# lambdaclass/lambdaworks_kzg

Measured on AMD Instinct MI355X. Metric: blob_to_kzg_commitment ops/sec (4096-elem blobs), higher is better.
Workload: dtype u32

## Files before the change

### lambdaworks_kzg_amd/csrc/direct.hip

```cpp
#include <stdlib.h>
#include <chrono>
#include "kernels.h"
#include "knobs.h"

namespace lwk {

template <int C>
struct DirectPlan {
    static constexpr int NW = (255 + C - 1) / C;
    static constexpr int H = 1 << (C - 1);
    static constexpr int WTOP = 255 - C * (NW - 1);
    static constexpr int HTOP = 1 << WTOP;
    static constexpr size_t TOP_BASE = (size_t)(NW - 1) * kBlobElems * H;
    static constexpr size_t ENTRIES = TOP_BASE + (size_t)kBlobElems * HTOP;
};

struct DirectPlanRt {
    int c, nw, wtop;
    uint32_t h, htop;
    size_t top_base, entries;
};

static DirectPlanRt make_plan(int bits) {
    DirectPlanRt p{};
// ... 382 lines not shown
    asm volatile(
#include "direct_fold_asm.inc"
        :
        : "s"(src), "s"(out), "s"(flag), "s"(per), "v"(lane), "s"(levels)
        :
#include "direct_fold_asm_clobbers.inc"
    );
#endif
}

__global__ __launch_bounds__(64) void k_direct_fold_lanes_asm_alone(const uint32_t *__restrict__ lane_out, G1Xyzz29 *__restrict__ partials,
                                                                    uint32_t *__restrict__ redo, int lanes_per_block, int blocks_per_blob) {
#if defined(__HIP_DEVICE_COMPILE__)
    const uint32_t unit = blockIdx.x;
    uint32_t *flag = redo + unit / blocks_per_blob;
    if (*flag) return;
    const uint32_t *src = lane_out + (size_t)unit * lanes_per_block * kLaneWords;
    G1Xyzz29 *out = partials + unit;
    const uint32_t per = lanes_per_block / 64, lane = threadIdx.x, levels = 6;
    asm volatile(
#include "direct_fold_asm.inc"
        :
        : "s"(src), "s"(out), "s"(flag), "s"(per), "v"(lane), "s"(levels)
        :
#include "direct_fold_asm_clobbers_pad.inc"
    );
#endif
}

template <bool ALONE>
__global__ __launch_bounds__(64) void k_commit_tail(const uint32_t *__restrict__ lane_out, G1Xyzz29 *__restrict__ sums,
                                                    uint32_t *__restrict__ redo, uint8_t *__restrict__ out48, int lanes_per_block) {
#if defined(__HIP_DEVICE_COMPILE__)
    const uint32_t blob = blockIdx.x;
    uint32_t *flag = redo + blob;
    G1Xyzz29 *out = sums + blob;
    const uint32_t lane = threadIdx.x;
    __builtin_amdgcn_s_setprio(2);
    if (!*flag) {
        const uint32_t *src = lane_out + (size_t)blob * lanes_per_block * kLaneWords;
        const uint32_t per = lanes_per_block / 64, levels = 6;
        if (ALONE) {
            asm volatile(
#include "direct_fold_asm.inc"
                :
                : "s"(src), "s"(out), "s"(flag), "s"(per), "v"(lane), "s"(levels)
                :
#include "direct_fold_asm_clobbers_pad.inc"
            );
        } else {
            asm volatile(
#include "direct_fold_asm.inc"
                :
                : "s"(src), "s"(out), "s"(flag), "s"(per), "v"(lane), "s"(levels)
                :
#include "direct_fold_asm_clobbers.inc"
            );
        }
        if (__hip_atomic_load(flag, __ATOMIC_RELAXED, __HIP_MEMORY_SCOPE_AGENT)) {
            const FoldPoint acc = fold_lane_sums(src + (size_t)lane * kLaneWords, (int)lane, (int)per);
            if (lane == 0) *out = *(const G1Xyzz29 *)&acc;
            __builtin_amdgcn_fence(__ATOMIC_RELEASE, "agent");
        }
    }
    uint32_t w[12];
    g1_compress_words(w, *out);
    if (lane != 0) return;
    uint32_t *o = (uint32_t *)(out48 + 48 * (size_t)blob);
#pragma unroll
    for (int k = 0; k < 12; k++) o[k] = w[k];
#endif
}

__global__ __launch_bounds__(64) void k_direct_fold(const G1Xyzz29 *__restrict__ partials, G1Xyzz29 *__restrict__ sums,
                                                    int per_blob) {
    const size_t b = blockIdx.x;
    const int lane = threadIdx.x;
    __builtin_amdgcn_s_setprio(2);
    G1Xyzz29 s = lane < per_blob ? partials[b * per_blob + lane] : G1Xyzz29::infinity();
    s = wave_fold(s, lane);
    if (lane == 0) sums[b] = s;
}

struct CoopParams {
    uint32_t k[8];
    uint32_t pack;
    uint32_t wtop, row_bytes, n0;
    uint32_t part_words, ctr_words;
};

constexpr uint32_t kCoopUnitWords = 56;

static void coop_geometry(const DirectPlanRt &P, int rpq, uint32_t &n0, uint32_t &units, uint32_t &counters) {
    const uint32_t groups = (uint32_t)((P.nw + rpq - 1) / rpq);
    n0 = kBlobElems * groups / 16;
    units = 0;
    counters = 0;
    for (uint32_t n = n0; n > 1; n = (n + 15) / 16) {
        units += n;
        counters += (n + 15) / 16;
    }
}

__global__ __launch_bounds__(256) void k_coop_msm_asm(const uint64_t *__restrict__ win_dev, const uint4 *__restrict__ scalars,
                                                     uint32_t *__restrict__ partials, uint32_t *__restrict__ counters,
                                                     G1Xyzz29 *__restrict__ sums, uint32_t *__restrict__ redo, CoopParams prm) {
#if defined(__HIP_DEVICE_COMPILE__)
    const uint32_t blob = blockIdx.y, lane = threadIdx.x & 63;
    const uint32_t unit = blockIdx.x * 4 + __builtin_amdgcn_readfirstlane(threadIdx.x >> 6);
    const uint4 *sc = scalars + (size_t)blob * kBlobElems * 2;
    uint32_t *part = partials + (size_t)blob * prm.part_words;
    uint32_t *ctr = counters + (size_t)blob * prm.ctr_words;
    G1Xyzz29 *out = sums + blob;
    uint32_t *flag = redo + blob;
    asm volatile(
#include "coop_asm.inc"
        :
        : "s"(win_dev), "s"(sc), "s"(part), "s"(ctr), "s"(out), "s"(flag), "s"(prm.k[0]), "s"(prm.k[1]), "s"(prm.k[2]), "s"(prm.k[3]),
          "s"(prm.k[4]), "s"(prm.k[5]), "s"(prm.k[6]), "s"(prm.k[7]), "s"(prm.pack), "s"(prm.wtop), "s"(prm.row_bytes), "s"(prm.n0), "s"(unit),
          "v"(lane)
        :
#include "coop_asm_clobbers.inc"
    );
#endif
}

static int coop_max_blobs() { return knobs().coop == 0 ? 0 : knobs().coop_max; }
static int coop_rows_per_quad(int nw, size_t n_blobs) {
    const int env = knobs().coop_rpq < 0 ? 0 : knobs().coop_rpq > 32 ? 32 : knobs().coop_rpq;
    if (env) return env;
    const int groups = n_blobs >= 4 ? 1 : (int)(4 / n_blobs);
    return (nw + groups - 1) / groups;
}

constexpr int kRedoRows = 256;
static bool direct_asm_enabled() { return knobs().direct_asm; }

template <int CT>
static bool launch_direct_t(const DirectPlanRt &plan, const uint64_t *table, size_t row_bytes, const uint32_t *scalars_raw,
                            G1Xyzz29 *lane_scratch, G1Xyzz29 *partials, uint32_t *redo, G1Xyzz29 *sums, size_t n_blobs, hipStream_t st,
                            int fill, uint32_t *redo_flag_out, uint8_t *out48 = nullptr, bool redo_cleared = false) {
    const int kFillEnv = knobs().direct_fill;
    const int kFill = kFillEnv ? kFillEnv : fill ? fill : 512;
    CoopParams prm{};
    const int rpq = coop_rows_per_quad(plan.nw, n_blobs ? n_blobs : 1);
    uint32_t units = 0, counters = 0;
    coop_geometry(plan, rpq, prm.n0, units, counters);
    const bool coop_fits = units <= (uint32_t)kBlobElems && 1 + counters <= (uint32_t)kNumBuckets + 1;
    if ((int)n_blobs <= coop_max_blobs() && !fill && coop_fits) {
        for (int j = 0; j + 1 < plan.nw; j++) {
            const int bit = plan.c * j;
            const uint64_t v = (uint64_t)(plan.h - 1) << (bit & 31);
            uint64_t carry = v;
            for (int w = bit >> 5; w < 8 && carry; w++) {
                carry += prm.k[w];
                prm.k[w] = (uint32_t)carry;
                carry >>= 32;
            }
        }
        prm.pack = (uint32_t)plan.c | ((uint32_t)plan.nw << 8) | ((uint32_t)rpq << 16) | (12u << 24);
        prm.wtop = (uint32_t)plan.wtop;
        prm.row_bytes = (uint32_t)row_bytes;
        prm.part_words = units * kCoopUnitWords;
        prm.ctr_words = counters;
        uint32_t *ctr = redo + n_blobs;
        if (redo_flag_out) {
            ProfScope p("k_coop_msm_asm", st);
            hipLaunchKernelGGL(k_coop_msm_asm, dim3(prm.n0 / 4, (unsigned)n_blobs), dim3(256), 0, st, table, (const uint4 *)scalars_raw,
                               (uint32_t *)lane_scratch, ctr, sums, redo_flag_out, prm);
            return false;
        }
        hipMemsetAsync(redo, 0, n_blobs * (1 + (size_t)counters) * sizeof(uint32_t), st);
        {
            ProfScope p("k_coop_msm_asm", st);
            hipLaunchKernelGGL(k_coop_msm_asm, dim3(prm.n0 / 4, (unsigned)n_blobs), dim3(256), 0, st, table, (const uint4 *)scalars_raw,
                               (uint32_t *)lane_scratch, ctr, sums, redo, prm);
        }
        {
            ProfScope p("k_direct_redo", st);
            hipLaunchKernelGGL(k_direct_accumulate<CT>, dim3(1, (unsigned)n_blobs, 1), dim3(kDirThreads), 0, st, table,
                               (const uint4 *)scalars_raw, sums, kBlobElems / kDirThreads, plan, (uint32_t)row_bytes, (const uint32_t *)redo);
        }
        return false;
    }
    int blocks_per_blob = 1, wsplit = 1;
    while (blocks_per_blob < 16 && n_blobs * blocks_per_blob < (size_t)kFill) blocks_per_blob <<= 1;
    while (wsplit < 4 && n_blobs * blocks_per_blob * wsplit * 8 <= (size_t)kFill) wsplit <<= 1;
    const int scalars_per_lane = kBlobElems / (kDirThreads * blocks_per_blob);
    const int parts = blocks_per_blob * wsplit;
    G1Xyzz29 *dest = parts == 1 ? sums : partials;
    if (out48 && direct_asm_enabled() && wsplit == 1 && blocks_per_blob == 1 && knobs().fold_asm && knobs().commit_tail) {
        if (!redo_cleared) hipMemsetAsync(redo, 0, n_blobs * sizeof(uint32_t), st);
        {
            ProfScope p("k_direct_accumulate_asm", st);
            hipLaunchKernelGGL(k_direct_accumulate_asm, dim3(1, (unsigned)n_blobs), dim3(kDirThreads), 0, st, table, (const uint4 *)scalars_raw,
                               (uint32_t *)lane_scratch, redo, kBlobElems / kDirThreads, plan, (uint32_t)row_bytes);
        }
        {
            ProfScope p("k_direct_redo", st);
            const unsigned rows = n_blobs < (size_t)kRedoRows ? (unsigned)n_blobs : (unsigned)kRedoRows;
            hipLaunchKernelGGL(k_direct_second_pass<CT>, dim3(1, rows, 1), dim3(kDirThreads), 0, st, table, (const uint4 *)scalars_raw, sums,
                               plan, (uint32_t)row_bytes, (const uint32_t *)redo, (uint32_t)n_blobs);
        }
        {
            ProfScope p("k_commit_tail", st);
            if (n_blobs >= 1024 && !fill)
                hipLaunchKernelGGL(k_commit_tail<true>, dim3((unsigned)n_blobs), dim3(64), 0, st, (const uint32_t *)lane_scratch, sums, redo, out48,
                                   kDirThreads);
            else
                hipLaunchKernelGGL(k_commit_tail<false>, dim3((unsigned)n_blobs), dim3(64), 0, st, (const uint32_t *)lane_scratch, sums, redo, out48,
                                   kDirThreads);
        }
        return true;
    }
    if (direct_asm_enabled() && wsplit == 1) {
        const int threads = kDirThreads;
        hipMemsetAsync(redo, 0, n_blobs * sizeof(uint32_t), st);
        {
            ProfScope p("k_direct_accumulate_asm", st);
            hipLaunchKernelGGL(k_direct_accumulate_asm, dim3(blocks_per_blob, (unsigned)n_blobs), dim3(threads), 0, st, table,
                               (const uint4 *)scalars_raw, (uint32_t *)lane_scratch, redo, kBlobElems / (threads * blocks_per_blob), plan,
                               (uint32_t)row_bytes);
        }
        {
            ProfScope p("k_direct_fold_lanes", st);
            const int n_units = (int)n_blobs * blocks_per_blob;
            const bool fold_asm = knobs().fold_asm;
            if (fold_asm) {
                if (n_units >= 1024 && !fill)
                    hipLaunchKernelGGL(k_direct_fold_lanes_asm_alone, dim3((unsigned)n_units), dim3(64), 0, st, (const uint32_t *)lane_scratch,
                                       dest, redo, threads, blocks_per_blob);
                else
                    hipLaunchKernelGGL(k_direct_fold_lanes_asm, dim3((unsigned)n_units), dim3(64), 0, st, (const uint32_t *)lane_scratch, dest,
                                       redo, threads, blocks_per_blob);
            } else {
                hipLaunchKernelGGL(k_direct_fold_lanes, dim3((unsigned)n_units), dim3(64), 0, st, (const uint32_t *)lane_scratch, dest,
                                   (const uint32_t *)redo, threads, blocks_per_blob);
            }
        }
        {
            ProfScope p("k_direct_redo", st);
            hipLaunchKernelGGL(k_direct_accumulate<CT>, dim3(blocks_per_blob, (unsigned)n_blobs, 1), dim3(kDirThreads), 0, st, table,
                               (const uint4 *)scalars_raw, dest, scalars_per_lane, plan, (uint32_t)row_bytes, (const uint32_t *)redo);
        }
    } else {
        ProfScope p("k_direct_accumulate", st);
        hipLaunchKernelGGL(k_direct_accumulate<CT>, dim3(blocks_per_blob, (unsigned)n_blobs, wsplit), dim3(kDirThreads), 0, st,
                           table, (const uint4 *)scalars_raw, dest, scalars_per_lane, plan, (uint32_t)row_bytes, (const uint32_t *)nullptr);
    }
    if (parts > 1) {
        ProfScope p("k_direct_fold", st);
        hipLaunchKernelGGL(k_direct_fold, dim3((unsigned)n_blobs), dim3(64), 0, st, partials, sums, parts);
    }
    return false;
}


static bool launch_direct_any(int bits, const uint64_t *table, size_t row_bytes, const uint32_t *scalars_raw, G1Xyzz29 *lane_scratch,
                              G1Xyzz29 *partials, uint32_t *redo, G1Xyzz29 *sums, size_t n_blobs, hipStream_t st, int fill, uint32_t *redo_flag_out,
                              uint8_t *out48, bool redo_cleared) {
    const DirectPlanRt plan = make_plan(bits);
    if (!plan.entries) return false;
    switch (bits) {
        case 14: return launch_direct_t<14>(plan, table, row_bytes, scalars_raw, lane_scratch, partials, redo, sums, n_blobs, st, fill, redo_flag_out, out48, redo_cleared);
        case 15: return launch_direct_t<15>(plan, table, row_bytes, scalars_raw, lane_scratch, partials, redo, sums, n_blobs, st, fill, redo_flag_out, out48, redo_cleared);
        case 16: return launch_direct_t<16>(plan, table, row_bytes, scalars_raw, lane_scratch, partials, redo, sums, n_blobs, st, fill, redo_flag_out, out48, redo_cleared);
        default: return launch_direct_t<0>(plan, table, row_bytes, scalars_raw, lane_scratch, partials, redo, sums, n_blobs, st, fill, redo_flag_out, out48, redo_cleared);
    }
}

void launch_direct_msm(int bits, const uint64_t *table, size_t row_bytes, const uint32_t *scalars_raw, G1Xyzz29 *lane_scratch,
                       G1Xyzz29 *partials, uint32_t *redo, G1Xyzz29 *sums, size_t n_blobs, hipStream_t st, int fill, uint32_t *redo_flag_out) {
    (void)launch_direct_any(bits, table, row_bytes, scalars_raw, lane_scratch, partials, redo, sums, n_blobs, st, fill, redo_flag_out, nullptr, false);
}

bool launch_direct_msm_compressed(int bits, const uint64_t *table, size_t row_bytes, const uint32_t *scalars_raw, G1Xyzz29 *lane_scratch,
                                  G1Xyzz29 *partials, uint32_t *redo, G1Xyzz29 *sums, uint8_t *out48, size_t n_blobs, hipStream_t st, int fill,
                                  bool redo_cleared) {
    return launch_direct_any(bits, table, row_bytes, scalars_raw, lane_scratch, partials, redo, sums, n_blobs, st, fill, nullptr, out48, redo_cleared);
}
uint32_t direct_one_blob_counter_words(int bits) {
    const DirectPlanRt plan = make_plan(bits);
    if (!plan.entries || coop_max_blobs() < 1) return 0;
    CoopParams prm{};
    uint32_t units = 0, counters = 0;
    coop_geometry(plan, coop_rows_per_quad(plan.nw, 1), prm.n0, units, counters);
    if (!(units <= (uint32_t)kBlobElems && 1 + counters <= (uint32_t)kNumBuckets + 1)) return 0;
    return counters;
}
template <int CT>
static void launch_direct_only_t(const DirectPlanRt &plan, const uint64_t *table, size_t row_bytes, const uint32_t *scalars_raw, G1Xyzz29 *sums,
                                 const uint32_t *only_if, size_t n_blobs, hipStream_t st) {
    ProfScope p("k_direct_redo", st);
    hipLaunchKernelGGL(k_direct_accumulate<CT>, dim3(1, (unsigned)n_blobs, 1), dim3(kDirThreads), 0, st, table, (const uint4 *)scalars_raw, sums,
                       kBlobElems / kDirThreads, plan, (uint32_t)row_bytes, only_if);
}

void launch_direct_msm_only(int bits, const uint64_t *table, size_t row_bytes, const uint32_t *scalars_raw, G1Xyzz29 *sums, const uint32_t *only_if,
                            size_t n_blobs, hipStream_t st) {
    const DirectPlanRt plan = make_plan(bits);
    if (!plan.entries) return;
    switch (bits) {
        case 14: launch_direct_only_t<14>(plan, table, row_bytes, scalars_raw, sums, only_if, n_blobs, st); break;
        case 15: launch_direct_only_t<15>(plan, table, row_bytes, scalars_raw, sums, only_if, n_blobs, st); break;
        case 16: launch_direct_only_t<16>(plan, table, row_bytes, scalars_raw, sums, only_if, n_blobs, st); break;
        default: launch_direct_only_t<0>(plan, table, row_bytes, scalars_raw, sums, only_if, n_blobs, st); break;
    }
}

}
```

### lambdaworks_kzg_amd/csrc/engine.hip

```cpp
#include "async_verifier.h"
#include "engine_internal.h"
#include "hostfp.h"

#include <stdarg.h>
#include <stdio.h>
#include <stdlib.h>
#include <string.h>

#include <atomic>
#include <chrono>
#include <map>
#include <set>
#include <thread>
#include <vector>

namespace lwk {


static thread_local char g_err[512] = "";

void set_error(const char *fmt, ...) {
    va_list ap;
    va_start(ap, fmt);
    vsnprintf(g_err, sizeof g_err, fmt, ap);
// ... 884 lines not shown
    C_KZG_RET rc = ctx_reserve(c, n);
    if (rc != C_KZG_OK) return rc;
    const bool longcall = n > kMaxChunk;
    if (longcall) {
        rc = ws_long_reserve(c, n);
        if (rc != C_KZG_OK) return rc;
    }
    Workspace &w = c->ws;
    const ModeRules mr = mode_rules(mode);
    const int le = mr.le(), fs = mr.hash_rule();
    int32_t *stt = status ? status : longcall ? w.status_long : w.status;
    Fr *z = longcall ? w.z_long : w.z;
    uint8_t *canon = longcall ? w.canon_long : w.canon48;
    LWK_HIP(hipMemsetAsync(stt, 0, n * 4, st));
    const bool evf = proof_in_evaluation_form(c, mode);
    const bool msm_direct = evf ? c->lag.direct_table != nullptr : c->direct_table && !proof_on_lagrange(c, mode);
    const bool warm = host_assist_warm(), busy = peer_busy(c);
    const PlanKnobs pk = plan_knobs();
    ProofPlan plan = plan_proof_call(n, warm, busy, msm_direct, true, pk);
    const int forced = knobs().proof_schedule;
    if (forced >= 0 && forced <= kProofGpuChains && n <= kMaxChunk) {
        PlanKnobs fk = pk;
        fk.small_proof_host = forced == kProofSmallHost ? kMaxChunk : 0;
        fk.mid_proof_host = forced == kProofSmallHost || forced == kProofGpuChains ? 0 : kMaxChunk;
        fk.mid_proof_pipe = forced == kProofMidPiped;
        fk.mid_proof_pipe_min = 0;
        plan = plan_proof_call(n, forced != kProofMidCold, false, forced == kProofMidPiped ? msm_direct : false, true, fk);
    }
    SmallProofArgs *host_args = nullptr;
    if (plan.needs_staging()) {
        bool ok = sph_reserve(c, n);
        if (ok && plan.schedule == kProofSmallHost) {
            host_args = new (std::nothrow) SmallProofArgs{&c->sph, n, mr.bad_status(), mr.be_transcript};
            ok = host_args != nullptr;
        }
        if (!ok) plan = plan_proof_call(n, warm, busy, msm_direct, false, pk);
    }
    g_last_proof_schedule.store((int)plan.schedule, std::memory_order_relaxed);
    const bool piped = plan.schedule == kProofMidPiped;
    switch (plan.schedule) {
    case kProofSmallHost: {
        SmallProofHost &h = c->sph;
        LWK_HIP(hipMemcpyAsync(h.blobs, blobs, n * (size_t)kBlobBytes, hipMemcpyDeviceToHost, st));
        LWK_HIP(hipMemcpyAsync(h.comm, comm48, n * 48, hipMemcpyDeviceToHost, st));
        {
            ProfScope p("host_challenge_and_validate", st);
            hipError_t e = hipLaunchHostFunc(st, small_proof_host_fn, host_args);
            if (e != hipSuccess) {
                delete host_args;
                set_error("hipLaunchHostFunc failed: %s", hipGetErrorString(e));
                return C_KZG_ERROR;
            }
        }
        LWK_HIP(hipMemcpyAsync(stt, h.code, n * 4, hipMemcpyHostToDevice, st));
        LWK_HIP(hipMemcpyAsync(w.zbytes, h.dig, n * 32, hipMemcpyHostToDevice, st));
        LWK_HIP(hipMemcpyAsync(canon, h.canon, n * 48, hipMemcpyHostToDevice, st));
        launch_z_from_bytes(w.zbytes, z, nullptr, le, n, st);
        launch_challenge(blobs, canon, z, fs, n, st, comm48);
        break;
    }
    case kProofMidCold: {
        LWK_HIP(hipEventRecord(c->ev_fork, st));
        LWK_HIP(hipStreamWaitEvent(c->vstream, c->ev_fork, 0));
        launch_validate_commitments(comm48, canon, stt, mr.bad_status(), n, c->vstream, longcall ? w.val_pts_long : w.val_pts,
                                    longcall ? w.val_kind_long : w.val_kind, longcall ? w.val_verdict_long : w.val_verdict);
        LWK_HIP(hipEventRecord(c->ev_join[0], c->vstream));
        launch_host_wake(c);
        launch_challenge(blobs, comm48, z, fs, n, st);
        LWK_HIP(hipStreamWaitEvent(st, c->ev_join[0], 0));
        launch_challenge(blobs, canon, z, fs, n, st, comm48);
        break;
    }
    case kProofMidHost:
    case kProofMidPiped: {
        SmallProofHost &h = c->sph;
        hipStream_t sc = c->aux[0], sh = c->aux[1];
        const size_t chunks = plan.chunks;
        LWK_HIP(hipEventRecord(c->ev_fork, st));
        LWK_HIP(hipStreamWaitEvent(c->vstream, c->ev_fork, 0));
        LWK_HIP(hipStreamWaitEvent(sc, c->ev_fork, 0));
        if (piped) LWK_HIP(hipStreamWaitEvent(sh, c->ev_fork, 0));
        launch_validate_commitments(comm48, canon, stt, mr.bad_status(), n, c->vstream, longcall ? w.val_pts_long : w.val_pts,
                                    longcall ? w.val_kind_long : w.val_kind, longcall ? w.val_verdict_long : w.val_verdict);
        LWK_HIP(hipEventRecord(c->ev_join[0], c->vstream));
        LWK_HIP(hipMemcpyAsync(h.comm, comm48, n * 48, hipMemcpyDeviceToHost, sc));
        {
            const C_KZG_RET rch = chunk_host_functions(c, blobs, n, sc, piped ? sh : st, st, chunk_hash_host_fn, "host_challenge_chunk", mr.be_transcript, piped);
            if (rch != C_KZG_OK) {
                hipStreamWaitEvent(st, c->ev_join[0], 0);
                return rch;
            }
        }
        if (piped) {
            const size_t per = plan.per_chunk;
            const size_t parts = plan.parts;
            const size_t cps = chunks / parts;
            uint32_t *differs = w.perm;
            hipStream_t s2 = c->aux[2];
            LWK_HIP(hipStreamWaitEvent(s2, c->ev_fork, 0));
            for (size_t j = 0; j < parts; j++) {
                const size_t off = j * cps * per, end_ = (j + 1) * cps * per < n ? (j + 1) * cps * per : n;
                if (off >= end_) continue;
                const size_t m = end_ - off;
                hipStream_t sk = (j & 1) ? s2 : st;
                LWK_HIP(hipStreamWaitEvent(sk, h.hashed[(j + 1) * cps - 1], 0));
                LWK_HIP(hipMemcpyAsync(w.zbytes + 32 * off, h.dig + 32 * off, m * 32, hipMemcpyHostToDevice, sk));
                launch_z_from_bytes(w.zbytes + 32 * off, z + off, nullptr, le, m, sk);
                coefficients_stage(c, blobs + off * (size_t)kBlobBytes, m, mode, stt + off, sk, off);
                quotient_stage(c, mode, w.scalars + off * (size_t)kBlobElems * 8, z + off, w.scalars2 + off * (size_t)kBlobElems * 8, nullptr, le, m, sk);
                (void)msm_sums_stage(c, w.scalars2 + off * (size_t)kBlobElems * 8, m, sk, off, false, evf);
            }
            LWK_HIP(hipEventRecord(c->ev_join[2], s2));
            LWK_HIP(hipStreamWaitEvent(st, c->ev_join[2], 0));
            LWK_HIP(hipStreamWaitEvent(st, c->ev_join[0], 0));
            launch_flag_differs48(canon, comm48, differs, n, st);
            launch_challenge(blobs, canon, z, fs, n, st, comm48);
            quotient_stage(c, mode, w.scalars, z, w.scalars2, nullptr, le, n, st, differs);
            launch_direct_msm_only(evf ? c->lag.direct_bits : c->direct_bits, evf ? c->lag.direct_tab.win_dev : c->direct_tab.win_dev,
                                   evf ? c->lag.direct_row_bytes : c->direct_row_bytes, w.scalars2, w.sums, differs, n, st);
            launch_finalize_compress(w.sums, out48, n, st);
            return C_KZG_OK;
        }
        LWK_HIP(hipMemcpyAsync(w.zbytes, h.dig, n * 32, hipMemcpyHostToDevice, st));
        launch_z_from_bytes(w.zbytes, z, nullptr, le, n, st);
        LWK_HIP(hipStreamWaitEvent(st, c->ev_join[0], 0));
        launch_challenge(blobs, canon, z, fs, n, st, comm48);
        break;
    }
    case kProofGpuChains: {
        LWK_HIP(hipEventRecord(c->ev_fork, st));
        LWK_HIP(hipStreamWaitEvent(c->vstream, c->ev_fork, 0));
        launch_validate_commitments(comm48, canon, stt, mr.bad_status(), n, c->vstream, longcall ? w.val_pts_long : w.val_pts,
                                    longcall ? w.val_kind_long : w.val_kind, longcall ? w.val_verdict_long : w.val_verdict);
        LWK_HIP(hipEventRecord(c->ev_join[0], c->vstream));
        launch_challenge(blobs, comm48, z, fs, n, st);
        LWK_HIP(hipStreamWaitEvent(st, c->ev_join[0], 0));
        launch_challenge(blobs, canon, z, fs, n, st, comm48);
        break;
    }
    }
    Ctx *pr = c->primary;
    const bool heavy_serial = plan.heavy_serial;
    if (heavy_serial) {
        std::lock_guard<std::mutex> hk(pr->heavy_mu);
        LWK_HIP(hipStreamWaitEvent(st, pr->heavy_done, 0));
    }
    for (size_t off = 0; off < n; off += kMaxChunk) {
        size_t m = n - off < kMaxChunk ? n - off : kMaxChunk;
        coefficients_stage(c, blobs + off * (size_t)kBlobBytes, m, mode, stt + off, st);
        quotient_stage(c, mode, w.scalars, z + off, w.scalars2, nullptr, le, m, st);
        G1Xyzz29 *sums = msm_sums_stage(c, w.scalars2, m, st, 0, false, quotient_to_msm_form(c, mode, m, st));
        if (heavy_serial && off + kMaxChunk >= n) {
            std::lock_guard<std::mutex> hk(pr->heavy_mu);
            LWK_HIP(hipEventRecord(pr->heavy_done, st));
        }
        launch_finalize_compress(sums, out48 + 48 * off, m, st);
    }
    return C_KZG_OK;
}

C_KZG_RET commit_and_prove_batch_device(Ctx *c, uint8_t *comm_out48, uint8_t *proof_out48, const uint8_t *blobs, size_t n, int mode,
                                        hipStream_t st, int32_t *status) {
    C_KZG_RET rc = ctx_reserve(c, n);
    if (rc != C_KZG_OK) return rc;
    const bool longcall = n > kMaxChunk;
    if (longcall) {
        rc = ws_long_reserve(c, n);
        if (rc != C_KZG_OK) return rc;
    }
    Workspace &w = c->ws;
    const ModeRules mr = mode_rules(mode);
    const int le = mr.le(), fs = mr.hash_rule();
    int32_t *stt = status ? status : longcall ? w.status_long : w.status;
    Fr *z = longcall ? w.z_long : w.z;
    uint32_t *mid = (uint32_t *)(longcall ? w.canon_long : w.canon48);
    LWK_HIP(hipMemsetAsync(stt, 0, n * 4, st));
    LWK_HIP(hipEventRecord(c->ev_fork, st));
    LWK_HIP(hipStreamWaitEvent(c->vstream, c->ev_fork, 0));
    const bool host_cold = n <= mid_proof_host_limit() && !peer_busy(c) && !host_assist_warm();
    if (host_cold) launch_host_wake(c);
    const bool host_mid = !host_cold && n <= mid_proof_host_limit() && !peer_busy(c) && sph_reserve(c, n);
    if (host_mid) {
        SmallProofHost &h = c->sph;
        hipStream_t sc = c->aux[0];
        LWK_HIP(hipStreamWaitEvent(sc, c->ev_fork, 0));
        {
            const C_KZG_RET rch = chunk_host_functions(c, blobs, n, sc, c->vstream, st, chunk_midstate_host_fn, "host_midstate_chunk", mr.be_transcript);
            if (rch != C_KZG_OK) return rch;
        }
        LWK_HIP(hipMemcpyAsync(mid, h.dig, n * 32, hipMemcpyHostToDevice, c->vstream));
    } else {
        launch_challenge_midstate(blobs, mid, n, c->vstream, mr.be_transcript);
    }
    LWK_HIP(hipEventRecord(c->ev_join[0], c->vstream));
    for (size_t off = 0; off < n; off += kMaxChunk) {
        const size_t m = n - off < kMaxChunk ? n - off : kMaxChunk;
        const uint8_t *b = blobs + off * (size_t)kBlobBytes;
        if (coefficients_stage(c, b, m, mode, stt + off, st)) {
            msm_stages(c, w.scalars, comm_out48 + 48 * off, m, st, 0, off == 0 && !host_mid, true);
        } else if (proof_on_lagrange(c, mode)) {
            if (le) launch_copy_le_check(b, (uint32_t *)w.fr, nullptr, m, st);
            else launch_copy_be_check(b, (uint32_t *)w.fr, nullptr, m, st);
            msm_stages(c, (const uint32_t *)w.fr, comm_out48 + 48 * off, m, st, 0, off == 0 && !host_mid, true);
        } else {
            msm_stages(c, w.scalars, comm_out48 + 48 * off, m, st, 0, off == 0 && !host_mid);
        }
        if (off == 0) LWK_HIP(hipStreamWaitEvent(st, c->ev_join[0], 0));
        launch_challenge_finish(b, comm_out48 + 48 * off, mid + 8 * off, z + off, fs, m, st);
        quotient_stage(c, mode, w.scalars, z + off, w.scalars2, nullptr, le, m, st);
        msm_stages(c, w.scalars2, proof_out48 + 48 * off, m, st, 0, false, quotient_to_msm_form(c, mode, m, st));
    }
    return C_KZG_OK;
}

C_KZG_RET point_proof_batch_device(Ctx *c, uint8_t *proof48, uint8_t *y32, const uint8_t *blobs, const uint8_t *z32,
                                   size_t n, int mode, hipStream_t st, int32_t *status, const G1Xyzz29 **sums_out) {
    C_KZG_RET rc = ctx_reserve(c, n);
    if (rc != C_KZG_OK) return rc;
    Workspace &w = c->ws;
    const ModeRules mr = mode_rules(mode);
    const int le = mr.le();
    for (size_t off = 0; off < n; off += kMaxChunk) {
        size_t m = n - off < kMaxChunk ? n - off : kMaxChunk;
        int32_t *stt = status ? status + off : w.status;
        LWK_HIP(hipMemsetAsync(stt, 0, m * 4, st));
        coefficients_stage(c, blobs + off * (size_t)kBlobBytes, m, mode, stt, st);
        launch_z_from_bytes(z32 + 32 * off, w.z, stt, mr.scalar_rule(), m, st);
        quotient_stage(c, mode, w.scalars, w.z, w.scalars2, y32 + 32 * off, le, m, st);
        const bool lg = quotient_to_msm_form(c, mode, m, st);
        if (sums_out && n <= kMaxChunk) *sums_out = msm_sums_stage(c, w.scalars2, m, st, 0, false, lg);
        else msm_stages(c, w.scalars2, proof48 + 48 * off, m, st, 0, false, lg);
    }
    return C_KZG_OK;
}

C_KZG_RET first_status(Ctx *c, const int32_t *d_status, size_t n, hipStream_t st) {
    std::vector<int32_t> h(n);
    LWK_HIP(hipMemcpyAsync(h.data(), d_status, n * 4, hipMemcpyDeviceToHost, st));
    LWK_HIP(hipStreamSynchronize(st));
// ... 126 lines not shown
```

### lambdaworks_kzg_amd/csrc/kernels.h

```cpp
#pragma once
#include <hip/hip_runtime.h>
#include <stdint.h>
#include "g1.cuh"
#include "fr28.cuh"
#include "plan.h"
#include "mode_rules.h"
#include "recover_sets.h"

namespace lwk {

struct ProfScope {
    ProfScope(const char *name, hipStream_t st);
    ~ProfScope();
    const char *name;
    hipStream_t st;
    hipEvent_t e0, e1;
    int dev;
    bool on;
};

void launch_parse_be_reduce(const uint8_t *blobs, uint32_t *scalars_raw, size_t n_elems, hipStream_t st, uint32_t *zero = nullptr, uint32_t zero_words = 0,
                            uint32_t *zero2 = nullptr, uint32_t zero2_words = 0);

void launch_digit_sort(const uint32_t *scalars_raw, uint32_t *sorted, uint32_t *bucket_start, uint32_t *perm,
                       size_t n_blobs, hipStream_t st);
void launch_bucket_accumulate(const G1Affine29 *table, const uint32_t *sorted, const uint32_t *bucket_start,
                              const uint32_t *perm, G1Xyzz29 *buckets, size_t n_blobs, hipStream_t st);
void launch_bucket_reduce(const G1Xyzz29 *buckets, G1Xyzz29 *sums, size_t n_blobs, hipStream_t st);
void launch_sum_points(const G1Xyzz29 *in, size_t n, G1Xyzz29 *total, int accumulate, hipStream_t st);
void launch_finalize_compress(const G1Xyzz29 *sums, uint8_t *out48, size_t n, hipStream_t st);

constexpr int kDirectMinBits = 10, kDirectMaxBits = 16;
constexpr size_t kDirectRowAligned = 128, kDirectRowPacked = 112;
constexpr size_t kDirectAlignedHeadroom = (size_t)8 << 30;
size_t direct_table_entries(int bits);
int direct_num_windows(int bits);
constexpr int kDirectMaxWindows = 26;
struct DirectTable {
    void *win[kDirectMaxWindows] = {};
    uint64_t *win_dev = nullptr;
    int nw = 0;
    size_t bytes = 0;
};
hipError_t build_direct_table(int bits, const G1Affine *points, DirectTable &table, size_t row_bytes, hipStream_t st, double *ms = nullptr,
                              bool in_place = false);
void free_direct_table(DirectTable &table);
void launch_direct_msm(int bits, const uint64_t *win_dev, size_t row_bytes, const uint32_t *scalars_raw, G1Xyzz29 *lane_scratch,
                       G1Xyzz29 *partials, uint32_t *redo, G1Xyzz29 *sums, size_t n_blobs, hipStream_t st, int fill = 0,
                       uint32_t *redo_flag_out = nullptr);
bool launch_direct_msm_compressed(int bits, const uint64_t *win_dev, size_t row_bytes, const uint32_t *scalars_raw, G1Xyzz29 *lane_scratch,
                                  G1Xyzz29 *partials, uint32_t *redo, G1Xyzz29 *sums, uint8_t *out48, size_t n_blobs, hipStream_t st,
                                  int fill = 0, bool redo_cleared = false);
uint32_t direct_one_blob_counter_words(int bits);
void launch_direct_msm_only(int bits, const uint64_t *win_dev, size_t row_bytes, const uint32_t *scalars_raw, G1Xyzz29 *sums,
                            const uint32_t *only_if, size_t n_blobs, hipStream_t st);

void launch_g1_decompress(const uint8_t *in48, G1Affine *out, int32_t *status, size_t n, int subgroup_check,
                          hipStream_t st);
void launch_g1_from_blst(const uint64_t *blst_p1, G1Affine *out, int32_t *status, size_t n, hipStream_t st);
void launch_g1_to_blst(const G1Affine *in, const int32_t *status, uint64_t *blst_p1, size_t n, hipStream_t st);
void launch_build_table(const G1Affine *points, G1Affine29 *table, hipStream_t st);

void launch_build_twiddles(Fr *tw_fwd, Fr *tw_inv, hipStream_t st);
void launch_twiddles_to28(const Fr *tw, Fr28 *tw28, hipStream_t st);
void launch_ntt4096(const Fr *in, Fr *out, const Fr28 *tw28, int inverse_scale_to_raw, size_t n_blobs, hipStream_t st);
void launch_blob_evaluations_to_coefficients(const uint8_t *blobs, uint32_t *coeffs_raw, const Fr28 *tw28_inv, int32_t *status,
                                             size_t n_blobs, hipStream_t st, int le = 1);
void launch_bitrev_permute(const Fr *in, Fr *out, size_t n_blobs, hipStream_t st);
void launch_idft_columns(uint32_t *coeffs_raw, const Fr *tw_inv, uint32_t first, size_t n_rows, hipStream_t st);
void launch_dft_rows(uint32_t *coeffs_raw, const Fr *tw_fwd, uint32_t first, size_t n_rows, hipStream_t st);
void launch_copy_le_check(const uint8_t *blobs, uint32_t *scalars_raw, int32_t *status, size_t n_blobs, hipStream_t st);
void launch_copy_be_check(const uint8_t *blobs, uint32_t *scalars_raw, int32_t *status, size_t n_blobs, hipStream_t st);
void launch_coefficients_to_evaluations(uint32_t *coeffs_raw, Fr *scratch, Fr *scratch2, const Fr28 *tw28_fwd, size_t n_blobs, hipStream_t st);
void launch_fr_be_to_mont(const uint8_t *in_be, Fr *out, size_t n_elems, hipStream_t st);
void launch_fr_mont_to_be(const Fr *in, uint8_t *out_be, size_t n_elems, hipStream_t st);
void launch_raw_to_be(const uint32_t *raw, uint8_t *out_be, size_t n_elems, hipStream_t st);
void launch_fr_mont_to_bytes(const Fr *in, uint8_t *out, int le, size_t n, hipStream_t st);
void launch_eval_quotient(const uint32_t *coeffs_raw, const Fr *z_mont, uint32_t *quot_raw, uint8_t *y_out, int le,
                          size_t n_blobs, hipStream_t st, const uint32_t *only_if = nullptr);
void launch_eval_y_from_blobs_be(const uint8_t *blobs, const Fr *z_mont, uint8_t *y_out, size_t n_blobs, hipStream_t st);
void launch_eval_y_from_blobs_evalform(const uint8_t *blobs, const Fr *z_mont, const Fr28 *roots_brp28, uint8_t *y_out, int32_t *status,
                                       size_t n_blobs, hipStream_t st, int le = 1);
void launch_roots_brp28(const Fr28 *tw28_fwd, Fr28 *roots_brp28, hipStream_t st);
void launch_eval_quotient_evalform(const uint32_t *evals_raw, const Fr *z_mont, const Fr28 *roots_brp28, uint32_t *quot_raw, uint8_t *y_out, int le,
                                   size_t n_blobs, hipStream_t st, const uint32_t *only_if = nullptr);
void launch_flag_differs48(const uint8_t *a, const uint8_t *b, uint32_t *flags, size_t n, hipStream_t st);
void launch_z_from_bytes(const uint8_t *z_bytes, Fr *z_mont, int32_t *status, int scalar_rule, size_t n, hipStream_t st);

struct PointSet {
    const uint8_t *in48;
    G1Affine29 *pts;
    int32_t *kind;
    uint8_t *canon48;
    uint32_t *verdict;
};
void launch_validate_commitments(const uint8_t *comm48, uint8_t *canon48, int32_t *status, int bad_code, size_t n,
                                 hipStream_t st, G1Affine29 *aff_out = nullptr, int32_t *kind_out = nullptr, uint32_t *verdict_scratch = nullptr,
                                 bool apart = false);
void launch_decompress_points(const PointSet &a, const PointSet *b, size_t n, hipStream_t st, bool apart = false);
void launch_subgroup_canon(const PointSet &a, const PointSet *b, int32_t *status, int bad_code, size_t n, hipStream_t st, bool apart = false);

size_t lincomb3_blocks(size_t n);
void launch_point_multiples(const G1Affine29 *pts_a, const int32_t *kind_a, G1Affine29 *mult_a, size_t n, hipStream_t st,
                            const G1Affine29 *pts_b = nullptr, const int32_t *kind_b = nullptr, G1Affine29 *mult_b = nullptr);
void launch_lincomb3(const G1Affine29 *proofs, const int32_t *proof_kind, const G1Affine29 *proof_mult, const G1Affine29 *comms,
                     const int32_t *comm_kind, const G1Affine29 *comm_mult, const uint8_t *sc_r_be, const uint8_t *sc_rz_be,
                     G1Xyzz29 *partial, size_t n, hipStream_t st);
constexpr int kVmsmDigits = 16;
constexpr int kVmsmRows = 2 * kVmsmDigits;
constexpr int kVmsmSteps = kVmsmDigits - 1;
constexpr int kVmsmMaxTerms = 64;
constexpr size_t kVmsmPinBytes = 33 * 32 + 3 * 96 + 3 * 4 + 52;
constexpr size_t kVmsmPinSums = 33 * 32, kVmsmPinInfs = kVmsmPinSums + 3 * 96, kVmsmPinSkip = kVmsmPinInfs + 3 * 4, kVmsmPinYsum = kVmsmPinSkip + 4;
static_assert(kVmsmPinYsum + 32 <= kVmsmPinBytes, "the asynchronous verification's words fit the pinned block");
constexpr int kVmsmPwSkip = 33, kVmsmPwYsum = 34, kVmsmPwSlots = 35;
constexpr int kVmsmListCap = 24;
void launch_vmsm_multiples2(const G1Affine29 *pts_a, const int32_t *kind_a, G1Affine29 *tab_a, const G1Affine29 *pts_b,
                            const int32_t *kind_b, G1Affine29 *tab_b, G1Xyzz29 *tmp, F29<2> *pre, size_t n, hipStream_t st, bool apart = false);
void launch_vmsm_scalars(const uint8_t *z_bytes, int le, const Fr *pw, uint32_t *sc_a, uint32_t *sc_b, size_t n, hipStream_t st,
                         const uint32_t *skip = nullptr);
uint32_t vmsm_terms_per_slice(size_t n);
size_t vmsm_slices(size_t n);
size_t vmsm_max_slices(size_t cap);
void launch_vmsm_accumulate(const uint32_t *sc_a, const uint32_t *sc_b, const G1Affine29 *tab_p, const int32_t *kind_p,
                            const G1Affine29 *tab_c, const int32_t *kind_c, G1Xyzz29 *partial, size_t n, hipStream_t st,
                            const uint32_t *sc_c = nullptr, const uint32_t *skip = nullptr);
void launch_vmsm_reduce(const G1Xyzz29 *partial, G1Xyzz29 *bsum, uint8_t *out96, int32_t *inf, size_t n, hipStream_t st,
                        const uint32_t *skip = nullptr);
void launch_verify_ysum(const uint8_t *y32, int le, const Fr *pw, uint8_t *out32, size_t n, hipStream_t st, const uint32_t *skip = nullptr);
void launch_verify_records(const uint8_t *canon_c, const uint8_t *z32, const uint8_t *y32, const uint8_t *canon_p, const int32_t *status,
                           uint8_t *records, uint32_t *first_bad, size_t n, hipStream_t st);
void launch_each_openings(const uint8_t *z_in, const uint8_t *y_in, uint8_t *z_out, uint8_t *y_out, int32_t *status, int bad_code,
                          int scalar_rule, size_t n, hipStream_t st);
void launch_xyzz29_to_affine_be(const G1Xyzz29 *in, uint8_t *out96, int32_t *inf, size_t n, hipStream_t st);

void launch_challenge(const uint8_t *blobs, const uint8_t *canon48, Fr *z_mont, int hash_rule, size_t n, hipStream_t st,
                      const uint8_t *only_if_differs_from = nullptr);
void launch_challenge_midstate(const uint8_t *blobs, uint32_t *midstate, size_t n, hipStream_t st, bool be_fields = false);
// ... 78 lines not shown
```

### lambdaworks_kzg_amd/csrc/msm.hip

```cpp
#include "kernels.h"
#include "knobs.h"

#include <stdlib.h>

namespace lwk {


__device__ __forceinline__ uint32_t bswap32(uint32_t v) { return __builtin_bswap32(v); }

__global__ __launch_bounds__(256) void k_parse_be_reduce(const uint4 *__restrict__ in, uint4 *__restrict__ out,
                                                         size_t n_elems, uint32_t *__restrict__ zero, uint32_t zero_words,
                                                         uint32_t *__restrict__ zero2, uint32_t zero2_words) {
    size_t i = (size_t)blockIdx.x * blockDim.x + threadIdx.x;
    if (i < zero_words) zero[i] = 0u;
    if (i < zero2_words) zero2[i] = 0u;
    if (i >= n_elems) return;
    uint4 hi = in[2 * i], lo = in[2 * i + 1];
    uint32_t s[8];
    s[7] = bswap32(hi.x);
    s[6] = bswap32(hi.y);
    s[5] = bswap32(hi.z);
    s[4] = bswap32(hi.w);
    s[3] = bswap32(lo.x);
    s[2] = bswap32(lo.y);
// ... 352 lines not shown
    sh[t] = run;
    __syncthreads();
    for (int d = 1; d < kRedThreads; d <<= 1) {
        G1Xyzz29 other = (t + d < kRedThreads) ? sh[t + d] : G1Xyzz29::infinity();
        __syncthreads();
        run = xyzz_add(run, other);
        sh[t] = run;
        __syncthreads();
    }
    sh[t] = (t >= 1) ? run : G1Xyzz29::infinity();
    __syncthreads();
    for (int d = kRedThreads / 2; d >= 1; d >>= 1) {
        if (t < d) sh[t] = xyzz_add(sh[t], sh[t + d]);
        __syncthreads();
    }
    G1Xyzz29 hi = sh[0];
    __syncthreads();
    sh[t] = wsum;
    __syncthreads();
    for (int d = kRedThreads / 2; d >= 1; d >>= 1) {
        if (t < d) sh[t] = xyzz_add(sh[t], sh[t + d]);
        __syncthreads();
    }
    if (t == 0) {
        for (int k = 1; k < kBucketsPerRedThread; k <<= 1) hi = xyzz_dbl(hi);
        sums[blob] = xyzz_add(sh[0], hi);
    }
}

static int reduce_lanes_override() {
    return knobs().reduce_lanes;
}

void launch_bucket_reduce(const G1Xyzz29 *buckets, G1Xyzz29 *sums, size_t n_blobs, hipStream_t st) {
    ProfScope p("k_bucket_reduce", st);
    int lanes = reduce_lanes_override();
    if (lanes == 0) lanes = n_blobs <= 256 ? 512 : 128;
    if (lanes >= 512)
        hipLaunchKernelGGL(k_bucket_reduce<512>, dim3((unsigned)n_blobs), dim3(512), 0, st, buckets, sums);
    else if (lanes >= 128)
        hipLaunchKernelGGL(k_bucket_reduce<128>, dim3((unsigned)n_blobs), dim3(128), 0, st, buckets, sums);
    else
        hipLaunchKernelGGL(k_bucket_reduce<64>, dim3((unsigned)n_blobs), dim3(64), 0, st, buckets, sums);
}


constexpr int kSumThreads = 256;

__global__ __launch_bounds__(kSumThreads) void k_sum_points(const G1Xyzz29 *__restrict__ in, size_t n,
                                                            G1Xyzz29 *__restrict__ total, int accumulate) {
    __shared__ G1Xyzz29 sh[kSumThreads];
    const int t = threadIdx.x;
    G1Xyzz29 acc = G1Xyzz29::infinity();
    for (size_t i = t; i < n; i += kSumThreads) acc = xyzz_add(acc, in[i]);
    sh[t] = acc;
    __syncthreads();
    for (int d = kSumThreads / 2; d >= 1; d >>= 1) {
        if (t < d) sh[t] = xyzz_add(sh[t], sh[t + d]);
        __syncthreads();
    }
    if (t == 0) total[0] = accumulate ? xyzz_add(total[0], sh[0]) : sh[0];
}

void launch_sum_points(const G1Xyzz29 *in, size_t n, G1Xyzz29 *total, int accumulate, hipStream_t st) {
    ProfScope p("k_sum_points", st);
    hipLaunchKernelGGL(k_sum_points, dim3(1), dim3(kSumThreads), 0, st, in, n, total, accumulate);
}


__global__ __launch_bounds__(64) void k_finalize_compress(const G1Xyzz29 *__restrict__ sums, uint8_t *__restrict__ out48,
                                                          size_t n) {
    size_t i = (size_t)blockIdx.x * blockDim.x + threadIdx.x;
    if (i >= n) return;
    __builtin_amdgcn_s_setprio(2);
    uint8_t b[48];
    g1_compress(b, sums[i]);
    uint32_t *o = (uint32_t *)(out48 + 48 * i);
#pragma unroll
    for (int k = 0; k < 12; k++)
        o[k] = (uint32_t)b[4 * k] | ((uint32_t)b[4 * k + 1] << 8) | ((uint32_t)b[4 * k + 2] << 16) |
               ((uint32_t)b[4 * k + 3] << 24);
}

void launch_finalize_compress(const G1Xyzz29 *sums, uint8_t *out48, size_t n, hipStream_t st) {
    ProfScope p("k_finalize_compress", st);
    hipLaunchKernelGGL(k_finalize_compress, dim3((unsigned)((n + 63) / 64)), dim3(64), 0, st, sums, out48, n);
}

}
```

Measured before the change: 115,800.

## Fuse partial fold and redo MSM with commitment compression into tail kernels

Adds kernels that fold per-blob partial sums and compress straight to 48-byte output, plus a redo-only MSM kernel that compresses after accumulating. This removes the separate finalize_compress launch in the commit paths when commit_tail is on. It also moves the differs check earlier onto the validation stream, and adds a wave-per-point finalize kernel for small batches. The cost is extra kernel variants and a cross-block fence that the fused redo path relies on for correctness.

```diff
diff --git a/lambdaworks_kzg_amd/csrc/direct.hip b/lambdaworks_kzg_amd/csrc/direct.hip
--- a/lambdaworks_kzg_amd/csrc/direct.hip
+++ b/lambdaworks_kzg_amd/csrc/direct.hip
@@ -488,6 +488,52 @@
     if (lane == 0) sums[b] = s;
 }
 
+__device__ __forceinline__ void wave_compress_store(const G1Xyzz29 &sum, uint8_t *__restrict__ out48, size_t index, int lane) {
+    uint32_t w[12];
+    g1_compress_words(w, sum);
+    if (lane != 0) return;
+    uint32_t *o = (uint32_t *)(out48 + 48 * index);
+#pragma unroll
+    for (int k = 0; k < 12; k++) o[k] = w[k];
+}
+
+__global__ __launch_bounds__(64) void k_direct_fold_compress(const G1Xyzz29 *__restrict__ partials, G1Xyzz29 *__restrict__ sums,
+                                                             const uint32_t *__restrict__ redo, uint8_t *__restrict__ out48, int per_blob,
+                                                             int width) {
+    const size_t b = blockIdx.x;
+    const int lane = threadIdx.x;
+    __builtin_amdgcn_s_setprio(2);
+    G1Xyzz29 s;
+    if (redo && redo[b]) {
+        s = sums[b];
+    } else {
+        s = lane < per_blob ? partials[b * per_blob + lane] : G1Xyzz29::infinity();
+        s = wave_fold(s, lane, width);
+        if (lane == 0) sums[b] = s;
+        G1Xyzz29i &t = *(G1Xyzz29i *)&s;
+#pragma unroll
+        for (int k = 0; k < 14; k++) {
+            t.x.l[k] = __shfl(t.x.l[k], 0, 64);
+            t.y.l[k] = __shfl(t.y.l[k], 0, 64);
+            t.zz.l[k] = __shfl(t.zz.l[k], 0, 64);
+            t.zzz.l[k] = __shfl(t.zzz.l[k], 0, 64);
+        }
+    }
+    wave_compress_store(s, out48, b, lane);
+}
+
+template <int CT>
+__global__ __launch_bounds__(kDirThreads) void k_direct_only_compress(const uint64_t *__restrict__ win_dev, const uint4 *__restrict__ scalars,
+                                                                      G1Xyzz29 *__restrict__ sums, DirectPlanRt rt, uint32_t row_bytes,
+                                                                      const uint32_t *__restrict__ only_if, uint8_t *__restrict__ out48) {
+    const size_t blob = blockIdx.y;
+    if (!only_if[blob]) return;
+    direct_accumulate_blob<CT>(win_dev, scalars, sums, kBlobElems / kDirThreads, rt, row_bytes, blob);
+    if (threadIdx.x >= 64) return;
+    __builtin_amdgcn_fence(__ATOMIC_SEQ_CST, "agent");
+    wave_compress_store(sums[blob], out48, blob, (int)threadIdx.x);
+}
+
 struct CoopParams {
     uint32_t k[8];
     uint32_t pack;
@@ -595,6 +641,8 @@
     const int scalars_per_lane = kBlobElems / (kDirThreads * blocks_per_blob);
     const int parts = blocks_per_blob * wsplit;
     G1Xyzz29 *dest = parts == 1 ? sums : partials;
+    const bool fused = out48 && parts > 1 && knobs().commit_tail;
+    const uint32_t *fused_redo = nullptr;
     if (out48 && direct_asm_enabled() && wsplit == 1 && blocks_per_blob == 1 && knobs().fold_asm && knobs().commit_tail) {
         if (!redo_cleared) hipMemsetAsync(redo, 0, n_blobs * sizeof(uint32_t), st);
         {
@@ -644,7 +692,13 @@
                                    (const uint32_t *)redo, threads, blocks_per_blob);
             }
         }
-        {
+        if (fused) {
+            ProfScope p("k_direct_redo", st);
+            const unsigned rows = n_blobs < (size_t)kRedoRows ? (unsigned)n_blobs : (unsigned)kRedoRows;
+            hipLaunchKernelGGL(k_direct_second_pass<CT>, dim3(1, rows, 1), dim3(kDirThreads), 0, st, table, (const uint4 *)scalars_raw, sums,
+                               plan, (uint32_t)row_bytes, (const uint32_t *)redo, (uint32_t)n_blobs);
+            fused_redo = redo;
+        } else {
             ProfScope p("k_direct_redo", st);
             hipLaunchKernelGGL(k_direct_accumulate<CT>, dim3(blocks_per_blob, (unsigned)n_blobs, 1), dim3(kDirThreads), 0, st, table,
                                (const uint4 *)scalars_raw, dest, scalars_per_lane, plan, (uint32_t)row_bytes, (const uint32_t *)redo);
@@ -653,6 +707,11 @@
         ProfScope p("k_direct_accumulate", st);
         hipLaunchKernelGGL(k_direct_accumulate<CT>, dim3(blocks_per_blob, (unsigned)n_blobs, wsplit), dim3(kDirThreads), 0, st,
                            table, (const uint4 *)scalars_raw, dest, scalars_per_lane, plan, (uint32_t)row_bytes, (const uint32_t *)nullptr);
+    }
+    if (fused) {
+        ProfScope p("k_direct_fold", st);
+        hipLaunchKernelGGL(k_direct_fold_compress, dim3((unsigned)n_blobs), dim3(64), 0, st, partials, sums, fused_redo, out48, parts, parts);
+        return true;
     }
     if (parts > 1) {
         ProfScope p("k_direct_fold", st);
@@ -696,22 +755,27 @@
 }
 template <int CT>
 static void launch_direct_only_t(const DirectPlanRt &plan, const uint64_t *table, size_t row_bytes, const uint32_t *scalars_raw, G1Xyzz29 *sums,
-                                 const uint32_t *only_if, size_t n_blobs, hipStream_t st) {
+                                 const uint32_t *only_if, size_t n_blobs, hipStream_t st, uint8_t *out48) {
     ProfScope p("k_direct_redo", st);
+    if (out48) {
+        hipLaunchKernelGGL(k_direct_only_compress<CT>, dim3(1, (unsigned)n_blobs, 1), dim3(kDirThreads), 0, st, table, (const uint4 *)scalars_raw,
+                           sums, plan, (uint32_t)row_bytes, only_if, out48);
+        return;
+    }
     hipLaunchKernelGGL(k_direct_accumulate<CT>, dim3(1, (unsigned)n_blobs, 1), dim3(kDirThreads), 0, st, table, (const uint4 *)scalars_raw, sums,
                        kBlobElems / kDirThreads, plan, (uint32_t)row_bytes, only_if);
 }
 
 void launch_direct_msm_only(int bits, const uint64_t *table, size_t row_bytes, const uint32_t *scalars_raw, G1Xyzz29 *sums, const uint32_t *only_if,
-                            size_t n_blobs, hipStream_t st) {
+                            size_t n_blobs, hipStream_t st, uint8_t *out48) {
     const DirectPlanRt plan = make_plan(bits);
     if (!plan.entries) return;
     switch (bits) {
-        case 14: launch_direct_only_t<14>(plan, table, row_bytes, scalars_raw, sums, only_if, n_blobs, st); break;
-        case 15: launch_direct_only_t<15>(plan, table, row_bytes, scalars_raw, sums, only_if, n_blobs, st); break;
-        case 16: launch_direct_only_t<16>(plan, table, row_bytes, scalars_raw, sums, only_if, n_blobs, st); break;
-        default: launch_direct_only_t<0>(plan, table, row_bytes, scalars_raw, sums, only_if, n_blobs, st); break;
-    }
-}
-
-}
+        case 14: launch_direct_only_t<14>(plan, table, row_bytes, scalars_raw, sums, only_if, n_blobs, st, out48); break;
+        case 15: launch_direct_only_t<15>(plan, table, row_bytes, scalars_raw, sums, only_if, n_blobs, st, out48); break;
+        case 16: launch_direct_only_t<16>(plan, table, row_bytes, scalars_raw, sums, only_if, n_blobs, st, out48); break;
+        default: launch_direct_only_t<0>(plan, table, row_bytes, scalars_raw, sums, only_if, n_blobs, st, out48); break;
+    }
+}
+
+}
diff --git a/lambdaworks_kzg_amd/csrc/engine.hip b/lambdaworks_kzg_amd/csrc/engine.hip
--- a/lambdaworks_kzg_amd/csrc/engine.hip
+++ b/lambdaworks_kzg_amd/csrc/engine.hip
@@ -990,6 +990,8 @@
         if (piped) LWK_HIP(hipStreamWaitEvent(sh, c->ev_fork, 0));
         launch_validate_commitments(comm48, canon, stt, mr.bad_status(), n, c->vstream, longcall ? w.val_pts_long : w.val_pts,
                                     longcall ? w.val_kind_long : w.val_kind, longcall ? w.val_verdict_long : w.val_verdict);
+        const bool differs_early = piped && knobs().commit_tail;
+        if (differs_early) launch_flag_differs48(canon, comm48, w.perm, n, c->vstream);
         LWK_HIP(hipEventRecord(c->ev_join[0], c->vstream));
         LWK_HIP(hipMemcpyAsync(h.comm, comm48, n * 48, hipMemcpyDeviceToHost, sc));
         {
@@ -1005,6 +1007,7 @@
             const size_t cps = chunks / parts;
             uint32_t *differs = w.perm;
             hipStream_t s2 = c->aux[2];
+            const bool tail = knobs().commit_tail;
             LWK_HIP(hipStreamWaitEvent(s2, c->ev_fork, 0));
             for (size_t j = 0; j < parts; j++) {
                 const size_t off = j * cps * per, end_ = (j + 1) * cps * per < n ? (j + 1) * cps * per : n;
@@ -1016,17 +1019,18 @@
                 launch_z_from_bytes(w.zbytes + 32 * off, z + off, nullptr, le, m, sk);
                 coefficients_stage(c, blobs + off * (size_t)kBlobBytes, m, mode, stt + off, sk, off);
                 quotient_stage(c, mode, w.scalars + off * (size_t)kBlobElems * 8, z + off, w.scalars2 + off * (size_t)kBlobElems * 8, nullptr, le, m, sk);
-                (void)msm_sums_stage(c, w.scalars2 + off * (size_t)kBlobElems * 8, m, sk, off, false, evf);
+                if (tail) msm_stages(c, w.scalars2 + off * (size_t)kBlobElems * 8, out48 + 48 * off, m, sk, off, false, evf);
+                else (void)msm_sums_stage(c, w.scalars2 + off * (size_t)kBlobElems * 8, m, sk, off, false, evf);
             }
             LWK_HIP(hipEventRecord(c->ev_join[2], s2));
             LWK_HIP(hipStreamWaitEvent(st, c->ev_join[2], 0));
             LWK_HIP(hipStreamWaitEvent(st, c->ev_join[0], 0));
-            launch_flag_differs48(canon, comm48, differs, n, st);
+            if (!differs_early) launch_flag_differs48(canon, comm48, differs, n, st);
             launch_challenge(blobs, canon, z, fs, n, st, comm48);
             quotient_stage(c, mode, w.scalars, z, w.scalars2, nullptr, le, n, st, differs);
             launch_direct_msm_only(evf ? c->lag.direct_bits : c->direct_bits, evf ? c->lag.direct_tab.win_dev : c->direct_tab.win_dev,
-                                   evf ? c->lag.direct_row_bytes : c->direct_row_bytes, w.scalars2, w.sums, differs, n, st);
-            launch_finalize_compress(w.sums, out48, n, st);
+                                   evf ? c->lag.direct_row_bytes : c->direct_row_bytes, w.scalars2, w.sums, differs, n, st, tail ? out48 : nullptr);
+            if (!tail) launch_finalize_compress(w.sums, out48, n, st);
             return C_KZG_OK;
         }
         LWK_HIP(hipMemcpyAsync(w.zbytes, h.dig, n * 32, hipMemcpyHostToDevice, st));
@@ -1057,12 +1061,15 @@
         size_t m = n - off < kMaxChunk ? n - off : kMaxChunk;
         coefficients_stage(c, blobs + off * (size_t)kBlobBytes, m, mode, stt + off, st);
         quotient_stage(c, mode, w.scalars, z + off, w.scalars2, nullptr, le, m, st);
-        G1Xyzz29 *sums = msm_sums_stage(c, w.scalars2, m, st, 0, false, quotient_to_msm_form(c, mode, m, st));
+        const bool lg = quotient_to_msm_form(c, mode, m, st);
+        G1Xyzz29 *sums = nullptr;
+        if (knobs().commit_tail) msm_stages(c, w.scalars2, out48 + 48 * off, m, st, 0, false, lg);
+        else sums = msm_sums_stage(c, w.scalars2, m, st, 0, false, lg);
         if (heavy_serial && off + kMaxChunk >= n) {
             std::lock_guard<std::mutex> hk(pr->heavy_mu);
             LWK_HIP(hipEventRecord(pr->heavy_done, st));
         }
-        launch_finalize_compress(sums, out48 + 48 * off, m, st);
+        if (sums) launch_finalize_compress(sums, out48 + 48 * off, m, st);
     }
     return C_KZG_OK;
 }
diff --git a/lambdaworks_kzg_amd/csrc/kernels.h b/lambdaworks_kzg_amd/csrc/kernels.h
--- a/lambdaworks_kzg_amd/csrc/kernels.h
+++ b/lambdaworks_kzg_amd/csrc/kernels.h
@@ -53,7 +53,7 @@
                                   int fill = 0, bool redo_cleared = false);
 uint32_t direct_one_blob_counter_words(int bits);
 void launch_direct_msm_only(int bits, const uint64_t *win_dev, size_t row_bytes, const uint32_t *scalars_raw, G1Xyzz29 *sums,
-                            const uint32_t *only_if, size_t n_blobs, hipStream_t st);
+                            const uint32_t *only_if, size_t n_blobs, hipStream_t st, uint8_t *out48 = nullptr);
 
 void launch_g1_decompress(const uint8_t *in48, G1Affine *out, int32_t *status, size_t n, int subgroup_check,
                           hipStream_t st);
diff --git a/lambdaworks_kzg_amd/csrc/msm.hip b/lambdaworks_kzg_amd/csrc/msm.hip
--- a/lambdaworks_kzg_amd/csrc/msm.hip
+++ b/lambdaworks_kzg_amd/csrc/msm.hip
@@ -458,8 +458,25 @@
                ((uint32_t)b[4 * k + 3] << 24);
 }
 
+__global__ __launch_bounds__(64) void k_finalize_compress_wave(const G1Xyzz29 *__restrict__ sums, uint8_t *__restrict__ out48) {
+    const size_t i = blockIdx.x;
+    __builtin_amdgcn_s_setprio(2);
+    uint32_t w[12];
+    g1_compress_words(w, sums[i]);
+    if (threadIdx.x != 0) return;
+    uint32_t *o = (uint32_t *)(out48 + 48 * i);
+#pragma unroll
+    for (int k = 0; k < 12; k++) o[k] = w[k];
+}
+
+constexpr size_t kFinalizeWaveMax = 1024;
+
 void launch_finalize_compress(const G1Xyzz29 *sums, uint8_t *out48, size_t n, hipStream_t st) {
     ProfScope p("k_finalize_compress", st);
+    if (n <= kFinalizeWaveMax && knobs().commit_tail) {
+        if (n) hipLaunchKernelGGL(k_finalize_compress_wave, dim3((unsigned)n), dim3(64), 0, st, sums, out48);
+        return;
+    }
     hipLaunchKernelGGL(k_finalize_compress, dim3((unsigned)((n + 63) / 64)), dim3(64), 0, st, sums, out48, n);
 }
 
```

New measurement: 114,500. 1.1% lower.
